# themattinthehatt/behavenet

Hardware: AMD Instinct MI355X
Metric: AE training frames/sec (128x128x1, batch 256) (higher is better)
Workload: dtype f32; 1 GPU; configs[1]: conv AE default arch, 1x128x128 f32 frames resident in HBM, 12 latents, batch 256 (chunks 200+56), fwd+bwd+Adam(amsgrad)

## Files before the change

### behavenet_amd/csrc/conv_qgemm2.hip

```cpp
#include <stdlib.h>
#include "bn_common.h"
#include "bn_fast.h"

typedef float q2x16 __attribute__((ext_vector_type(16)));
typedef float q2x4 __attribute__((ext_vector_type(4)));

#define Q2_THREADS 256
#define Q2_OOB 0x7fffffff
#define Q2_MAX_LDS (160 * 1024)

__device__ __forceinline__ void q2_dma16(__amdgpu_buffer_rsrc_t rsrc, char* lds, int voffset,
                                         int soffset) {
    __builtin_amdgcn_raw_ptr_buffer_load_lds(rsrc, (float*)lds, 16, voffset, soffset, 0, 0);
}

#define Q2_R0(z) (((z) >> 1) ? 0 : 1)
#define Q2_S0(z) (((z) & 1) ? 0 : 1)

#define Q2U_KS 32
#define Q2U_PAIR 1040
#define Q2U_SBYTES (16 * Q2U_PAIR)
#define Q2U_WROW 200
#define Q2U_WINSTR 25
#define Q2U_WBYTES (Q2U_WINSTR * 1024)
#define Q2U_STAGE (Q2U_SBYTES + Q2U_WBYTES)
#define Q2U_NDMA 11

__global__ __launch_bounds__(Q2_THREADS, 1) void k_qg2_up(
    const float* __restrict__ small, const float* __restrict__ w, const float* __restrict__ bias,
    float* __restrict__ out, const float* __restrict__ dact_src, int N, int Cs, int Cb, int act,
    int dact, float slope) {
    extern __shared__ __attribute__((aligned(16))) char smem[];
    const int tid = threadIdx.x, lane = tid & 63;
    const int wv = __builtin_amdgcn_readfirstlane(tid >> 6);
    const int li = lane & 31, kh = lane >> 5;
    const int cw0 = blockIdx.x * 8, c0 = cw0 + 2 * wv, n0 = blockIdx.y * 32;

    const __amdgpu_buffer_rsrc_t rs_s = __builtin_amdgcn_make_buffer_rsrc(
        (void*)small, 0, (int)((size_t)N * Cs * 16), 0x00020000);
    const __amdgpu_buffer_rsrc_t rs_w = __builtin_amdgcn_make_buffer_rsrc(
        (void*)w, 0, (int)((size_t)Cs * Cb * 100), 0x00020000);

    const int vo_s = ((n0 + (lane >> 5)) * Cs + (lane & 31)) * 16;
    int vo_w[7];
#pragma unroll
    for (int h = 0; h < 7; ++h) {
        const int grp = 64 * (wv + 4 * h) + lane;
        const int ml = grp / 50, gi = grp - 50 * ml;
        vo_w[h] = (ml * Cb + cw0) * 100 + gi * 16;
    }
    auto issue_dma = [&](const int d, const int buf, const int stage) __attribute__((always_inline)) {
        char* base = smem + buf * Q2U_STAGE;
        if (d < 4) {
            q2_dma16(rs_s, base + (4 * wv + d) * Q2U_PAIR, vo_s, (2 * (4 * wv + d) * Cs + stage * Q2U_KS) * 16);
        } else {
            const int h = d - 4;
            if (wv + 4 * h < Q2U_WINSTR)
                q2_dma16(rs_w, base + Q2U_SBYTES + (wv + 4 * h) * 1024, vo_w[h], stage * Q2U_KS * Cb * 100);
        }
    };

    const int ad_s = (li >> 1) * Q2U_PAIR + ((li & 1) * 32 + kh) * 16;
    const int jj = li & 15;
    const int ad_w = Q2U_SBYTES + (kh * Q2U_WROW + (2 * wv + (li >> 4)) * 25 + (jj >> 2) * 5 + (jj & 3)) * 4;

    q2x16 acc[4];
#pragma unroll
    for (int z = 0; z < 4; ++z)
#pragma unroll
        for (int t = 0; t < 16; ++t) acc[z][t] = 0.f;

    const int n_stages = Cs / Q2U_KS;
#pragma unroll
    for (int d = 0; d < Q2U_NDMA; ++d) issue_dma(d, 0, 0);

#ifdef Q2U_LOOP_SHIFT
    BN_LOOP_PLACE(8, Q2U_LOOP_SHIFT);
#endif
    for (int st = 0; st < n_stages; ++st) {
        asm volatile("s_waitcnt vmcnt(0)" ::: "memory");
        __syncthreads();
        const int buf = st & 1;
#ifdef Q2_ABL_NODMA
        const bool more = false;
#else
        const bool more = st + 1 < n_stages;
#endif
        const char* sp = smem + buf * Q2U_STAGE + ad_s;
        int wo[4];
#pragma unroll
        for (int z = 0; z < 4; ++z) {
            wo[z] = buf * Q2U_STAGE + ad_w + (Q2_R0(z) * 5 + Q2_S0(z)) * 4;
            asm volatile("" : "+v"(wo[z]));
        }
        q2x4 sv[2];
        float wq[2][4];
        sv[0] = *reinterpret_cast<const q2x4*>(sp);
#pragma unroll
        for (int z = 0; z < 4; ++z) wq[0][z] = *reinterpret_cast<const float*>(smem + wo[z]);
#pragma unroll
        for (int t = 0; t < 16; ++t) {
            const int cu = t & 1, nx = cu ^ 1;
            if (t + 1 < 16) {
                sv[nx] = *reinterpret_cast<const q2x4*>(sp + (t + 1) * 32);
#pragma unroll
                for (int z = 0; z < 4; ++z)
                    wq[nx][z] = *reinterpret_cast<const float*>(smem + wo[z] + (t + 1) * 2 * Q2U_WROW * 4);
            }
            __builtin_amdgcn_sched_barrier(0);
            acc[0] = __builtin_amdgcn_mfma_f32_32x32x2f32(wq[cu][0], sv[cu].x, acc[0], 0, 0, 0);
            acc[1] = __builtin_amdgcn_mfma_f32_32x32x2f32(wq[cu][1], sv[cu].y, acc[1], 0, 0, 0);
            if (more && t < Q2U_NDMA) issue_dma(t, buf ^ 1, st + 1);
            acc[2] = __builtin_amdgcn_mfma_f32_32x32x2f32(wq[cu][2], sv[cu].z, acc[2], 0, 0, 0);
            acc[3] = __builtin_amdgcn_mfma_f32_32x32x2f32(wq[cu][3], sv[cu].w, acc[3], 0, 0, 0);
            __builtin_amdgcn_sched_barrier(0);
        }
    }

    const int n = n0 + li;
    const int obytes = (int)((size_t)N * Cb * 64 * 4);
    const __amdgpu_buffer_rsrc_t ro = __builtin_amdgcn_make_buffer_rsrc((void*)out, 0, obytes, 0x00020000);
    const __amdgpu_buffer_rsrc_t rd = __builtin_amdgcn_make_buffer_rsrc(
        (void*)dact_src, 0, dact_src ? obytes : 0, 0x00020000);
    const int vo = (n < N) ? (n * Cb + c0) * 256 : Q2_OOB;
    const float es = (act == BN_ACT_LRELU) ? slope : 1.f;
    const float ds = (dact == BN_ACT_LRELU) ? slope : 1.f;
    float bz[2] = {0.f, 0.f};
    if (bias) { bz[0] = bias[c0]; bz[1] = bias[c0 + 1]; }
#pragma unroll
    for (int z = 0; z < 4; ++z) {
        q2x4 d[4];
#pragma unroll
        for (int tq = 0; tq < 4; ++tq) {
            const int so = (tq >> 1) * 256 + ((4 * (z >> 1) + 2 * (tq & 1)) * 8 + 4 * (z & 1)) * 4;
            if (dact_src)
                d[tq] = __builtin_bit_cast(q2x4, __builtin_amdgcn_raw_buffer_load_b128(rd, vo + kh * 32, so, 0));
        }
#pragma unroll
        for (int tq = 0; tq < 4; ++tq) {
            const int so = (tq >> 1) * 256 + ((4 * (z >> 1) + 2 * (tq & 1)) * 8 + 4 * (z & 1)) * 4;
            q2x4 v;
#pragma unroll
            for (int e = 0; e < 4; ++e) {
                float x = acc[z][4 * tq + e] + bz[tq >> 1];
                x = x > 0.f ? x : x * es;
                if (dact_src) x *= d[tq][e] > 0.f ? 1.f : ds;
                v[e] = x;
            }
            __builtin_amdgcn_raw_buffer_store_b128(__builtin_bit_cast(__attribute__((ext_vector_type(4))) unsigned int, v),
                                                   ro, vo + kh * 32, so, 0);
        }
    }
}

bool bn_qg2_up_supported(const BnGeom& g, int act, int dact) {
    if (!bn_qgemm_supported(g)) return false;
    if (act == BN_ACT_SIGMOID || dact == BN_ACT_SIGMOID) return false;
    if ((g.Cs % Q2U_KS) != 0 || (g.Cb & 7) != 0) return false;
    if (((g.N + 31) / 32) * (g.Cb / 8) < 128) return false;
    return true;
}

int bn_launch_qg2_up(const float* small, const float* w, const float* bias, float* out,
                     const float* dact_src, const BnGeom& g, int act, int dact, float slope,
                     hipStream_t st) {
    static bool attr_set = false;
    if (!attr_set) {
        hipError_t e = hipFuncSetAttribute((const void*)k_qg2_up, hipFuncAttributeMaxDynamicSharedMemorySize,
                                           Q2_MAX_LDS);
        if (e != hipSuccess) return (int)e;
        attr_set = true;
    }
    const dim3 grid(g.Cb / 8, (g.N + 31) / 32);
    BN_LAUNCH_MAIN(k_qg2_up, grid, dim3(Q2_THREADS), (size_t)2 * Q2U_STAGE, st, small, w, bias, out,
                   dact_src, g.N, g.Cs, g.Cb, act, dact, slope);
    BN_LAUNCH_CHECK();
    return 0;
}

#define Q2W_KS 16
#define Q2W_SBYTES (Q2W_KS * 1024)
#define Q2W_BBYTES (Q2W_KS * 2048)
#define Q2W_STAGE (Q2W_SBYTES + Q2W_BBYTES)
#define Q2W_NBUF 3
#define Q2W_NDMA 12

__global__ __launch_bounds__(Q2_THREADS, 1) void k_qg2_wgrad(
    const float* __restrict__ small, const float* __restrict__ big, float* __restrict__ dw,
    float* __restrict__ db, int N, int Cs, int Cb, int accumulate, int bias_side) {
    extern __shared__ __attribute__((aligned(16))) char smem[];
    const int tid = threadIdx.x, lane = tid & 63;
    const int wv = __builtin_amdgcn_readfirstlane(tid >> 6);
    const int li = lane & 31, kh = lane >> 5;
    const int mb = wv & 1, cq = wv >> 1;
    const int c0 = blockIdx.x * 8, m0 = blockIdx.y * 64;

    const __amdgpu_buffer_rsrc_t rs_s = __builtin_amdgcn_make_buffer_rsrc(
        (void*)small, 0, (int)((size_t)N * Cs * 16), 0x00020000);
    const __amdgpu_buffer_rsrc_t rs_b = __builtin_amdgcn_make_buffer_rsrc(
        (void*)big, 0, (int)((size_t)N * Cb * 256), 0x00020000);
    const int vo_s = (m0 + lane) * 16;
    const int vo_b = c0 * 256 + lane * 16;
    auto issue_dma = [&](const int d, const int buf, const int stage) __attribute__((always_inline)) {
        char* base = smem + buf * Q2W_STAGE;
        if (d < 4) {
            const int nl = 4 * wv + d;
            q2_dma16(rs_s, base + nl * 1024, vo_s, (stage * Q2W_KS + nl) * Cs * 16);
        } else {
            const int nl = 4 * wv + ((d - 4) >> 1), half = (d - 4) & 1;
            q2_dma16(rs_b, base + Q2W_SBYTES + nl * 2048 + half * 1024, vo_b,
                     (stage * Q2W_KS + nl) * Cb * 256 + half * 1024);
        }
    };

    const int jj = li & 15;
    const int ad_a = (kh * 64 + 32 * mb + li) * 16;
    const int ad_b = Q2W_SBYTES + (kh * 512 + (4 * cq + (li >> 4)) * 64 + (jj >> 2) * 8 + (jj & 3)) * 4;

    q2x16 acc[2][4];
#pragma unroll
    for (int cb = 0; cb < 2; ++cb)
#pragma unroll
        for (int z = 0; z < 4; ++z)
#pragma unroll
            for (int t = 0; t < 16; ++t) acc[cb][z][t] = 0.f;
    float bsum = 0.f;
    const bool do_bias1 = (bias_side == 1) && db && blockIdx.x == 0;
    const bool do_bias2 = (bias_side == 2) && db && blockIdx.y == 0;

    const int n_stages = (N + Q2W_KS - 1) / Q2W_KS;
#pragma unroll
    for (int d = 0; d < Q2W_NDMA; ++d) issue_dma(d, 0, 0);
    if (n_stages > 1) {
#pragma unroll
        for (int d = 0; d < Q2W_NDMA; ++d) issue_dma(d, 1, 1);
    }

    int buf = 0;
#ifdef Q2W_LOOP_SHIFT
    BN_LOOP_PLACE(8, Q2W_LOOP_SHIFT);
#endif
    for (int st = 0; st < n_stages; ++st) {
        if (st + 1 < n_stages) asm volatile("s_waitcnt vmcnt(12)" ::: "memory");
        else                   asm volatile("s_waitcnt vmcnt(0)" ::: "memory");
        __builtin_amdgcn_s_barrier();
        const bool more = st + 2 < n_stages;
        const int nbuf = (buf + 2 >= Q2W_NBUF) ? buf + 2 - Q2W_NBUF : buf + 2;
        const char* base = smem + buf * Q2W_STAGE;
        if (do_bias1) {
            const char* p = base + ((tid >> 6) * 4 * 64 + (tid & 63)) * 16;
#pragma unroll
            for (int i = 0; i < 4; ++i) {
                const q2x4 v = *reinterpret_cast<const q2x4*>(p + i * 1024);
                bsum += (v.x + v.y) + (v.z + v.w);
            }
        }
        if (do_bias2) {
            const char* p = base + Q2W_SBYTES + tid * 16;
#pragma unroll
            for (int i = 0; i < 8; ++i) {
                const q2x4 v = *reinterpret_cast<const q2x4*>(p + i * 4096);
                bsum += (v.x + v.y) + (v.z + v.w);
            }
        }
        const char* ap = base + ad_a;
        int bo[4];
#pragma unroll
        for (int z = 0; z < 4; ++z) {
            bo[z] = buf * Q2W_STAGE + ad_b + (32 * (z >> 1) + 4 * (z & 1)) * 4;
            asm volatile("" : "+v"(bo[z]));
        }
        q2x4 sv[2];
        float bq[2][2][4];
        sv[0] = *reinterpret_cast<const q2x4*>(ap);
#pragma unroll
        for (int cb = 0; cb < 2; ++cb)
#pragma unroll
            for (int z = 0; z < 4; ++z) bq[0][cb][z] = *reinterpret_cast<const float*>(smem + bo[z] + cb * 512);
#pragma unroll
        for (int t = 0; t < Q2W_KS / 2; ++t) {
            const int cu = t & 1, nx = cu ^ 1;
            if (t + 1 < Q2W_KS / 2) {
                sv[nx] = *reinterpret_cast<const q2x4*>(ap + (t + 1) * 2048);
#pragma unroll
                for (int cb = 0; cb < 2; ++cb)
#pragma unroll
                    for (int z = 0; z < 4; ++z)
                        bq[nx][cb][z] = *reinterpret_cast<const float*>(smem + bo[z] + cb * 512 + (t + 1) * 4096);
            }
            __builtin_amdgcn_sched_barrier(0);
#pragma unroll
            for (int z = 0; z < 4; ++z) {
                acc[0][z] = __builtin_amdgcn_mfma_f32_32x32x2f32(sv[cu][z], bq[cu][0][z], acc[0][z], 0, 0, 0);
                acc[1][z] = __builtin_amdgcn_mfma_f32_32x32x2f32(sv[cu][z], bq[cu][1][z], acc[1][z], 0, 0, 0);
                if (more && z < 2 && t < 6) issue_dma(2 * t + z, nbuf, st + 2);
            }
            __builtin_amdgcn_sched_barrier(0);
        }
        buf = (buf + 1 >= Q2W_NBUF) ? 0 : buf + 1;
    }

    float* P = reinterpret_cast<float*>(smem);
    float* R = reinterpret_cast<float*>(smem + 4 * 32 * 128 * 4);
    float* bred = reinterpret_cast<float*>(smem + 4 * 32 * 128 * 4 + 32 * 200 * 4);
    __syncthreads();
    if (do_bias1 || do_bias2) bred[tid] = bsum;
#pragma unroll 1
    for (int h = 0; h < 2; ++h) {
        if (mb == h) {
#pragma unroll
            for (int cb = 0; cb < 2; ++cb)
#pragma unroll
                for (int z = 0; z < 4; ++z)
#pragma unroll
                    for (int t = 0; t < 16; ++t) {
                        const int m = (t & 3) + 8 * (t >> 2) + 4 * kh;
                        P[(z * 32 + m) * 128 + 64 * cq + 32 * cb + li] = acc[cb][z][t];
                    }
        }
        __syncthreads();
        {
            const int m = tid >> 3, c = tid & 7;
            float q[4][16];
#pragma unroll
            for (int z = 0; z < 4; ++z)
#pragma unroll
                for (int g4 = 0; g4 < 4; ++g4) {
                    const q2x4 v = *reinterpret_cast<const q2x4*>(P + (z * 32 + m) * 128 + c * 16 + 4 * g4);
                    q[z][4 * g4 + 0] = v.x; q[z][4 * g4 + 1] = v.y; q[z][4 * g4 + 2] = v.z; q[z][4 * g4 + 3] = v.w;
                }
#pragma unroll
            for (int tap = 0; tap < 25; ++tap) {
                const int r = tap / 5, s = tap - 5 * r;
                float v = 0.f;
#pragma unroll
                for (int zp = 0; zp < 2; ++zp) {
                    const int yy = r - (zp ? 0 : 1);
                    if (yy < 0 || yy > 3) continue;
#pragma unroll
                    for (int zq = 0; zq < 2; ++zq) {
                        const int xx = s - (zq ? 0 : 1);
                        if (xx < 0 || xx > 3) continue;
                        v += q[2 * zp + zq][4 * yy + xx];
                    }
                }
                R[m * 200 + c * 25 + tap] = v;
            }
        }
        __syncthreads();
        for (int i = tid; i < 32 * 50; i += Q2_THREADS) {
            const int m = i / 50, g4 = i - 50 * m;
            q2x4 v = *reinterpret_cast<const q2x4*>(R + m * 200 + 4 * g4);
            float* dst = dw + ((size_t)(m0 + 32 * h + m) * Cb + c0) * 25 + 4 * g4;
            if (accumulate) {
                const q2x4 d = *reinterpret_cast<const q2x4*>(dst);
                v.x += d.x; v.y += d.y; v.z += d.z; v.w += d.w;
            }
            *reinterpret_cast<q2x4*>(dst) = v;
        }
    }
    if (do_bias1 && tid < 64) {
        const float v = ((bred[tid] + bred[64 + tid]) + bred[128 + tid]) + bred[192 + tid];
        db[m0 + tid] = accumulate ? db[m0 + tid] + v : v;
    }
    if (do_bias2 && tid < 8) {
        float v = 0.f;
        for (int par = 0; par < 2; ++par)
            for (int g4 = 0; g4 < 16; ++g4) v += bred[par * 128 + tid * 16 + g4];
        db[c0 + tid] = accumulate ? db[c0 + tid] + v : v;
    }
}

bool bn_qg2_wgrad_supported(const BnGeom& g) {
    if (!bn_qgemm_supported(g)) return false;
    return (g.Cs % 64) == 0 && (g.Cb % 8) == 0;
}

int bn_launch_qg2_wgrad(const float* small, const float* big, float* dw, const BnGeom& g,
                        int accumulate, float* db, int bias_side, hipStream_t st) {
    static bool attr_set = false;
    if (!attr_set) {
        hipError_t e = hipFuncSetAttribute((const void*)k_qg2_wgrad, hipFuncAttributeMaxDynamicSharedMemorySize,
                                           Q2_MAX_LDS);
        if (e != hipSuccess) return (int)e;
        attr_set = true;
    }
    const dim3 grid(g.Cb / 8, g.Cs / 64);
    BN_LAUNCH_MAIN(k_qg2_wgrad, grid, dim3(Q2_THREADS), (size_t)Q2W_NBUF * Q2W_STAGE, st, small, big, dw,
                   db, g.N, g.Cs, g.Cb, accumulate, bias_side);
    BN_LAUNCH_CHECK();
    return 0;
}
```

Before: 58610 frames/s.

## Split K across two wave groups in qgemm2 up and wgrad kernels

Doubles the block to 512 threads and splits each stage's K loop between two groups of four waves. Each group computes partial accumulators, and the halves are combined with an LDS exchange before the epilogue. DMA issue is redistributed across eight waves and the wait counts are adjusted to match. The aim is more waves per CU to hide MFMA and LDS latency, at the cost of an extra reduction pass through shared memory and more registers per block.

Result: no change. 58740 frames/s (median of 6 runs) (+0.2%).

```diff
diff --git a/behavenet_amd/csrc/conv_qgemm2.hip b/behavenet_amd/csrc/conv_qgemm2.hip
--- a/behavenet_amd/csrc/conv_qgemm2.hip
+++ b/behavenet_amd/csrc/conv_qgemm2.hip
@@ -5,7 +5,7 @@
 typedef float q2x16 __attribute__((ext_vector_type(16)));
 typedef float q2x4 __attribute__((ext_vector_type(4)));
 
-#define Q2_THREADS 256
+#define Q2_THREADS 512
 #define Q2_OOB 0x7fffffff
 #define Q2_MAX_LDS (160 * 1024)
 
@@ -18,13 +18,14 @@
 #define Q2_S0(z) (((z) & 1) ? 0 : 1)
 
 #define Q2U_KS 32
+#define Q2U_KSTEPS (Q2U_KS / 4)
 #define Q2U_PAIR 1040
 #define Q2U_SBYTES (16 * Q2U_PAIR)
 #define Q2U_WROW 200
 #define Q2U_WINSTR 25
 #define Q2U_WBYTES (Q2U_WINSTR * 1024)
 #define Q2U_STAGE (Q2U_SBYTES + Q2U_WBYTES)
-#define Q2U_NDMA 11
+#define Q2U_NDMA 6
 
 __global__ __launch_bounds__(Q2_THREADS, 1) void k_qg2_up(
     const float* __restrict__ small, const float* __restrict__ w, const float* __restrict__ bias,
@@ -34,7 +35,8 @@
     const int tid = threadIdx.x, lane = tid & 63;
     const int wv = __builtin_amdgcn_readfirstlane(tid >> 6);
     const int li = lane & 31, kh = lane >> 5;
-    const int cw0 = blockIdx.x * 8, c0 = cw0 + 2 * wv, n0 = blockIdx.y * 32;
+    const int wp = wv & 3, kg = wv >> 2;
+    const int cw0 = blockIdx.x * 8, c0 = cw0 + 2 * wp, n0 = blockIdx.y * 32;
 
     const __amdgpu_buffer_rsrc_t rs_s = __builtin_amdgcn_make_buffer_rsrc(
         (void*)small, 0, (int)((size_t)N * Cs * 16), 0x00020000);
@@ -42,27 +44,28 @@
         (void*)w, 0, (int)((size_t)Cs * Cb * 100), 0x00020000);
 
     const int vo_s = ((n0 + (lane >> 5)) * Cs + (lane & 31)) * 16;
-    int vo_w[7];
-#pragma unroll
-    for (int h = 0; h < 7; ++h) {
-        const int grp = 64 * (wv + 4 * h) + lane;
+    int vo_w[4];
+#pragma unroll
+    for (int h = 0; h < 4; ++h) {
+        const int grp = 64 * (wv + 8 * h) + lane;
         const int ml = grp / 50, gi = grp - 50 * ml;
         vo_w[h] = (ml * Cb + cw0) * 100 + gi * 16;
     }
     auto issue_dma = [&](const int d, const int buf, const int stage) __attribute__((always_inline)) {
         char* base = smem + buf * Q2U_STAGE;
-        if (d < 4) {
-            q2_dma16(rs_s, base + (4 * wv + d) * Q2U_PAIR, vo_s, (2 * (4 * wv + d) * Cs + stage * Q2U_KS) * 16);
+        if (d < 2) {
+            q2_dma16(rs_s, base + (2 * wv + d) * Q2U_PAIR, vo_s, (2 * (2 * wv + d) * Cs + stage * Q2U_KS) * 16);
         } else {
-            const int h = d - 4;
-            if (wv + 4 * h < Q2U_WINSTR)
-                q2_dma16(rs_w, base + Q2U_SBYTES + (wv + 4 * h) * 1024, vo_w[h], stage * Q2U_KS * Cb * 100);
+            const int h = d - 2;
+            if (wv + 8 * h < Q2U_WINSTR)
+                q2_dma16(rs_w, base + Q2U_SBYTES + (wv + 8 * h) * 1024, vo_w[h], stage * Q2U_KS * Cb * 100);
         }
     };
 
-    const int ad_s = (li >> 1) * Q2U_PAIR + ((li & 1) * 32 + kh) * 16;
+    const int ad_s = (li >> 1) * Q2U_PAIR + ((li & 1) * 32 + kh) * 16 + kg * Q2U_KSTEPS * 32;
     const int jj = li & 15;
-    const int ad_w = Q2U_SBYTES + (kh * Q2U_WROW + (2 * wv + (li >> 4)) * 25 + (jj >> 2) * 5 + (jj & 3)) * 4;
+    const int ad_w = Q2U_SBYTES + ((kh + 2 * kg * Q2U_KSTEPS) * Q2U_WROW + (2 * wp + (li >> 4)) * 25 +
+                                   (jj >> 2) * 5 + (jj & 3)) * 4;
 
     q2x16 acc[4];
 #pragma unroll
@@ -99,9 +102,9 @@
 #pragma unroll
         for (int z = 0; z < 4; ++z) wq[0][z] = *reinterpret_cast<const float*>(smem + wo[z]);
 #pragma unroll
-        for (int t = 0; t < 16; ++t) {
+        for (int t = 0; t < Q2U_KSTEPS; ++t) {
             const int cu = t & 1, nx = cu ^ 1;
-            if (t + 1 < 16) {
+            if (t + 1 < Q2U_KSTEPS) {
                 sv[nx] = *reinterpret_cast<const q2x4*>(sp + (t + 1) * 32);
 #pragma unroll
                 for (int z = 0; z < 4; ++z)
@@ -110,45 +113,72 @@
             __builtin_amdgcn_sched_barrier(0);
             acc[0] = __builtin_amdgcn_mfma_f32_32x32x2f32(wq[cu][0], sv[cu].x, acc[0], 0, 0, 0);
             acc[1] = __builtin_amdgcn_mfma_f32_32x32x2f32(wq[cu][1], sv[cu].y, acc[1], 0, 0, 0);
-            if (more && t < Q2U_NDMA) issue_dma(t, buf ^ 1, st + 1);
+            if (more && 2 * t < Q2U_NDMA) issue_dma(2 * t, buf ^ 1, st + 1);
             acc[2] = __builtin_amdgcn_mfma_f32_32x32x2f32(wq[cu][2], sv[cu].z, acc[2], 0, 0, 0);
             acc[3] = __builtin_amdgcn_mfma_f32_32x32x2f32(wq[cu][3], sv[cu].w, acc[3], 0, 0, 0);
+            if (more && 2 * t + 1 < Q2U_NDMA) issue_dma(2 * t + 1, buf ^ 1, st + 1);
             __builtin_amdgcn_sched_barrier(0);
         }
+    }
+
+    q2x16 fin[2];
+    {
+        q2x4* X = reinterpret_cast<q2x4*>(smem);
+        __syncthreads();
+        q2x4* xo = X + (wv * 8) * 64 + lane;
+#pragma unroll
+        for (int zi = 0; zi < 2; ++zi)
+#pragma unroll
+            for (int tq = 0; tq < 4; ++tq) {
+                q2x4 v;
+#pragma unroll
+                for (int e = 0; e < 4; ++e) v[e] = kg ? acc[zi][4 * tq + e] : acc[2 + zi][4 * tq + e];
+                xo[(zi * 4 + tq) * 64] = v;
+            }
+        __syncthreads();
+        const q2x4* xi = X + ((wv ^ 4) * 8) * 64 + lane;
+#pragma unroll
+        for (int zi = 0; zi < 2; ++zi)
+#pragma unroll
+            for (int tq = 0; tq < 4; ++tq) {
+                const q2x4 v = xi[(zi * 4 + tq) * 64];
+#pragma unroll
+                for (int e = 0; e < 4; ++e)
+                    fin[zi][4 * tq + e] = kg ? v[e] + acc[2 + zi][4 * tq + e] : acc[zi][4 * tq + e] + v[e];
+            }
     }
 
     const int n = n0 + li;
     const int obytes = (int)((size_t)N * Cb * 64 * 4);
-    const __amdgpu_buffer_rsrc_t ro = __builtin_amdgcn_make_buffer_rsrc((void*)out, 0, obytes, 0x00020000);
     const __amdgpu_buffer_rsrc_t rd = __builtin_amdgcn_make_buffer_rsrc(
         (void*)dact_src, 0, dact_src ? obytes : 0, 0x00020000);
-    const int vo = (n < N) ? (n * Cb + c0) * 256 : Q2_OOB;
+    const int vo = ((n < N) ? (n * Cb + c0) * 256 : Q2_OOB) + kh * 32 + kg * 128;
+    float* const op = out + ((size_t)(n < N ? n : 0) * Cb + c0) * 64 + kh * 8 + kg * 32;
     const float es = (act == BN_ACT_LRELU) ? slope : 1.f;
     const float ds = (dact == BN_ACT_LRELU) ? slope : 1.f;
     float bz[2] = {0.f, 0.f};
     if (bias) { bz[0] = bias[c0]; bz[1] = bias[c0 + 1]; }
 #pragma unroll
-    for (int z = 0; z < 4; ++z) {
+    for (int zi = 0; zi < 2; ++zi) {
         q2x4 d[4];
 #pragma unroll
         for (int tq = 0; tq < 4; ++tq) {
-            const int so = (tq >> 1) * 256 + ((4 * (z >> 1) + 2 * (tq & 1)) * 8 + 4 * (z & 1)) * 4;
+            const int so = (tq >> 1) * 256 + (2 * (tq & 1) * 8 + 4 * zi) * 4;
             if (dact_src)
-                d[tq] = __builtin_bit_cast(q2x4, __builtin_amdgcn_raw_buffer_load_b128(rd, vo + kh * 32, so, 0));
+                d[tq] = __builtin_bit_cast(q2x4, __builtin_amdgcn_raw_buffer_load_b128(rd, vo, so, 0));
         }
 #pragma unroll
         for (int tq = 0; tq < 4; ++tq) {
-            const int so = (tq >> 1) * 256 + ((4 * (z >> 1) + 2 * (tq & 1)) * 8 + 4 * (z & 1)) * 4;
+            const int so = (tq >> 1) * 256 + (2 * (tq & 1) * 8 + 4 * zi) * 4;
             q2x4 v;
 #pragma unroll
             for (int e = 0; e < 4; ++e) {
-                float x = acc[z][4 * tq + e] + bz[tq >> 1];
+                float x = fin[zi][4 * tq + e] + bz[tq >> 1];
                 x = x > 0.f ? x : x * es;
                 if (dact_src) x *= d[tq][e] > 0.f ? 1.f : ds;
                 v[e] = x;
             }
-            __builtin_amdgcn_raw_buffer_store_b128(__builtin_bit_cast(__attribute__((ext_vector_type(4))) unsigned int, v),
-                                                   ro, vo + kh * 32, so, 0);
+            if (n < N) *reinterpret_cast<q2x4*>(op + so / 4) = v;
         }
     }
 }
@@ -183,7 +213,8 @@
 #define Q2W_BBYTES (Q2W_KS * 2048)
 #define Q2W_STAGE (Q2W_SBYTES + Q2W_BBYTES)
 #define Q2W_NBUF 3
-#define Q2W_NDMA 12
+#define Q2W_KSTEPS (Q2W_KS / 4)
+#define Q2W_NDMA 6
 
 __global__ __launch_bounds__(Q2_THREADS, 1) void k_qg2_wgrad(
     const float* __restrict__ small, const float* __restrict__ big, float* __restrict__ dw,
@@ -192,7 +223,7 @@
     const int tid = threadIdx.x, lane = tid & 63;
     const int wv = __builtin_amdgcn_readfirstlane(tid >> 6);
     const int li = lane & 31, kh = lane >> 5;
-    const int mb = wv & 1, cq = wv >> 1;
+    const int mb = wv & 1, cq = (wv >> 1) & 1, kg = wv >> 2;
     const int c0 = blockIdx.x * 8, m0 = blockIdx.y * 64;
 
     const __amdgpu_buffer_rsrc_t rs_s = __builtin_amdgcn_make_buffer_rsrc(
@@ -203,19 +234,19 @@
     const int vo_b = c0 * 256 + lane * 16;
     auto issue_dma = [&](const int d, const int buf, const int stage) __attribute__((always_inline)) {
         char* base = smem + buf * Q2W_STAGE;
-        if (d < 4) {
-            const int nl = 4 * wv + d;
+        if (d < 2) {
+            const int nl = 2 * wv + d;
             q2_dma16(rs_s, base + nl * 1024, vo_s, (stage * Q2W_KS + nl) * Cs * 16);
         } else {
-            const int nl = 4 * wv + ((d - 4) >> 1), half = (d - 4) & 1;
+            const int nl = 2 * wv + ((d - 2) >> 1), half = (d - 2) & 1;
             q2_dma16(rs_b, base + Q2W_SBYTES + nl * 2048 + half * 1024, vo_b,
                      (stage * Q2W_KS + nl) * Cb * 256 + half * 1024);
         }
     };
 
     const int jj = li & 15;
-    const int ad_a = (kh * 64 + 32 * mb + li) * 16;
-    const int ad_b = Q2W_SBYTES + (kh * 512 + (4 * cq + (li >> 4)) * 64 + (jj >> 2) * 8 + (jj & 3)) * 4;
+    const int ad_a = ((kh + 2 * kg * Q2W_KSTEPS) * 64 + 32 * mb + li) * 16;
+    const int ad_b = Q2W_SBYTES + ((kh + 2 * kg * Q2W_KSTEPS) * 512 + (4 * cq + (li >> 4)) * 64 + (jj >> 2) * 8 + (jj & 3)) * 4;
 
     q2x16 acc[2][4];
 #pragma unroll
@@ -241,16 +272,16 @@
     BN_LOOP_PLACE(8, Q2W_LOOP_SHIFT);
 #endif
     for (int st = 0; st < n_stages; ++st) {
-        if (st + 1 < n_stages) asm volatile("s_waitcnt vmcnt(12)" ::: "memory");
+        if (st + 1 < n_stages) asm volatile("s_waitcnt vmcnt(6)" ::: "memory");
         else                   asm volatile("s_waitcnt vmcnt(0)" ::: "memory");
         __builtin_amdgcn_s_barrier();
         const bool more = st + 2 < n_stages;
         const int nbuf = (buf + 2 >= Q2W_NBUF) ? buf + 2 - Q2W_NBUF : buf + 2;
         const char* base = smem + buf * Q2W_STAGE;
         if (do_bias1) {
-            const char* p = base + ((tid >> 6) * 4 * 64 + (tid & 63)) * 16;
-#pragma unroll
-            for (int i = 0; i < 4; ++i) {
+            const char* p = base + ((tid >> 6) * 2 * 64 + (tid & 63)) * 16;
+#pragma unroll
+            for (int i = 0; i < 2; ++i) {
                 const q2x4 v = *reinterpret_cast<const q2x4*>(p + i * 1024);
                 bsum += (v.x + v.y) + (v.z + v.w);
             }
@@ -258,8 +289,8 @@
         if (do_bias2) {
             const char* p = base + Q2W_SBYTES + tid * 16;
 #pragma unroll
-            for (int i = 0; i < 8; ++i) {
-                const q2x4 v = *reinterpret_cast<const q2x4*>(p + i * 4096);
+            for (int i = 0; i < 4; ++i) {
+                const q2x4 v = *reinterpret_cast<const q2x4*>(p + i * 8192);
                 bsum += (v.x + v.y) + (v.z + v.w);
             }
         }
@@ -278,9 +309,9 @@
 #pragma unroll
             for (int z = 0; z < 4; ++z) bq[0][cb][z] = *reinterpret_cast<const float*>(smem + bo[z] + cb * 512);
 #pragma unroll
-        for (int t = 0; t < Q2W_KS / 2; ++t) {
+        for (int t = 0; t < Q2W_KSTEPS; ++t) {
             const int cu = t & 1, nx = cu ^ 1;
-            if (t + 1 < Q2W_KS / 2) {
+            if (t + 1 < Q2W_KSTEPS) {
                 sv[nx] = *reinterpret_cast<const q2x4*>(ap + (t + 1) * 2048);
 #pragma unroll
                 for (int cb = 0; cb < 2; ++cb)
@@ -293,11 +324,38 @@
             for (int z = 0; z < 4; ++z) {
                 acc[0][z] = __builtin_amdgcn_mfma_f32_32x32x2f32(sv[cu][z], bq[cu][0][z], acc[0][z], 0, 0, 0);
                 acc[1][z] = __builtin_amdgcn_mfma_f32_32x32x2f32(sv[cu][z], bq[cu][1][z], acc[1][z], 0, 0, 0);
-                if (more && z < 2 && t < 6) issue_dma(2 * t + z, nbuf, st + 2);
+                if (more && z < 2 && 2 * t + z < Q2W_NDMA) issue_dma(2 * t + z, nbuf, st + 2);
             }
             __builtin_amdgcn_sched_barrier(0);
         }
         buf = (buf + 1 >= Q2W_NBUF) ? 0 : buf + 1;
+    }
+
+    q2x16 fin[4];
+    {
+        q2x4* X = reinterpret_cast<q2x4*>(smem);
+        __syncthreads();
+        q2x4* xo = X + (wv * 16) * 64 + lane;
+#pragma unroll
+        for (int z = 0; z < 4; ++z)
+#pragma unroll
+            for (int tq = 0; tq < 4; ++tq) {
+                q2x4 v;
+#pragma unroll
+                for (int e = 0; e < 4; ++e) v[e] = kg ? acc[0][z][4 * tq + e] : acc[1][z][4 * tq + e];
+                xo[(z * 4 + tq) * 64] = v;
+            }
+        __syncthreads();
+        const q2x4* xi = X + ((wv ^ 4) * 16) * 64 + lane;
+#pragma unroll
+        for (int z = 0; z < 4; ++z)
+#pragma unroll
+            for (int tq = 0; tq < 4; ++tq) {
+                const q2x4 v = xi[(z * 4 + tq) * 64];
+#pragma unroll
+                for (int e = 0; e < 4; ++e)
+                    fin[z][4 * tq + e] = kg ? v[e] + acc[1][z][4 * tq + e] : acc[0][z][4 * tq + e] + v[e];
+            }
     }
 
     float* P = reinterpret_cast<float*>(smem);
@@ -309,17 +367,15 @@
     for (int h = 0; h < 2; ++h) {
         if (mb == h) {
 #pragma unroll
-            for (int cb = 0; cb < 2; ++cb)
-#pragma unroll
-                for (int z = 0; z < 4; ++z)
-#pragma unroll
-                    for (int t = 0; t < 16; ++t) {
-                        const int m = (t & 3) + 8 * (t >> 2) + 4 * kh;
-                        P[(z * 32 + m) * 128 + 64 * cq + 32 * cb + li] = acc[cb][z][t];
-                    }
-        }
-        __syncthreads();
-        {
+            for (int z = 0; z < 4; ++z)
+#pragma unroll
+                for (int t = 0; t < 16; ++t) {
+                    const int m = (t & 3) + 8 * (t >> 2) + 4 * kh;
+                    P[(z * 32 + m) * 128 + 64 * cq + 32 * kg + li] = fin[z][t];
+                }
+        }
+        __syncthreads();
+        if (tid < 256) {
             const int m = tid >> 3, c = tid & 7;
             float q[4][16];
 #pragma unroll
@@ -360,12 +416,13 @@
         }
     }
     if (do_bias1 && tid < 64) {
-        const float v = ((bred[tid] + bred[64 + tid]) + bred[128 + tid]) + bred[192 + tid];
+        float v = 0.f;
+        for (int g8 = 0; g8 < 8; ++g8) v += bred[64 * g8 + tid];
         db[m0 + tid] = accumulate ? db[m0 + tid] + v : v;
     }
     if (do_bias2 && tid < 8) {
         float v = 0.f;
-        for (int par = 0; par < 2; ++par)
+        for (int par = 0; par < 4; ++par)
             for (int g4 = 0; g4 < 16; ++g4) v += bred[par * 128 + tid * 16 + g4];
         db[c0 + tid] = accumulate ? db[c0 + tid] + v : v;
     }
```
